# NikhilMukraj/spiking-neural-networks

Measured on AMD Instinct MI355X. Metric: neuron-steps/sec, higher is better.
Workload: dtype f32; 1 GPU; 256x256 Izhikevich lattice, dense gap-junction connectivity (all-to-all, x != y), dt=0.1, weights U[0.5,1.5]; neurons=65536, parallelism=single GPU

## Files before the change

### spiking-neural-networks_amd/csrc/snn_network_state.hpp

```cpp
#pragma once
#include <hip/hip_runtime.h>

#include <algorithm>
#include <atomic>
#include <cmath>
#include <cstdint>
#include <cstdio>
#include <cstdlib>
#include <cstring>
#include <map>
#include <memory>
#include <new>
#include <stdexcept>
#include <string>
#include <utility>
#include <vector>

#include "../../include/snn_amd.h"
#include "snn_kernels_connect.hpp"
#include "snn_kernels_connect_csr.hpp"
#include "snn_kernels_csr.hpp"
#include "snn_kernels_dense_step.hpp"
#include "snn_kernels_exchange.hpp"
#include "snn_kernels_graph_query.hpp"
// ... 128 lines not shown
    int plane;
    uint32_t pad;
    int dirties;
};

struct LatticeInfo {
    uint32_t id, rows, cols, first, count, slot;
    bool spike_train;
};

struct Cursors {
    long long clock = 0, run_step_offset = 0;
    uint64_t hist_steps = 0, hist_tick = 0;
};
struct CacheState {
    int shadow_cur = 0, cell_view_cur = 0;
    bool shadow_valid = false;
    bool view_dirty = true;
    bool counts_dirty = true, uni_dirty = true;
    uint32_t live_mask_applied = 0xFFFFFFFFu, n_live = K_TYPES, live_type[K_TYPES] = {0, 1, 2};
    uint32_t mirror_mask = 0xFFFFFFFFu;
};
struct Stats {
    struct Run { uint64_t launches = 0, steps = 0, stdp_steps = 0; } run;
    uint64_t run_fallbacks = 0, run_external_stream = 0;
    uint64_t direct_steps = 0, peer_steps = 0;
    uint64_t steps_dense_one_launch = 0, steps_dense_close = 0, steps_sparse_one_launch = 0, steps_sparse_image = 0;
    uint64_t steps_sparse_split = 0, steps_two_kernel = 0;
    uint64_t shadow_refreshes = 0, view_refreshes = 0, history_regrows = 0;
    uint64_t verify_runs = 0, verify_mismatches = 0, verify_skipped = 0;
};

}

struct snn_network {
    int device = 0;
    Options opt;
    Stats stat;
    Cursors cur;
    CacheState cache;
    hipStream_t stream = nullptr;
    hipStream_t own_stream = nullptr;
    bool external_stream = false;
    int model = 0, nt_kind = 0, rc_kind = 0, st_kind = 0;
    bool finalized = false;
    int electrical = 1, chemical = 0;

    hvec<LatticeInfo> lattices;
    hvec<LatticeInfo> st_lattices;
    hvec<long long> st_clock;
    hvec<float> stdp_host;
    hvec<uint32_t> plast_host;
    bool any_plasticity = false;
    std::map<uint32_t, bool> lattice_has_nt;
    bool any_nt_neurons = false, any_nt_cells = false;
    std::map<uint32_t, uint32_t> lattice_nt_mask;
    bool any_modulation = false;
    bool any_modulated = false;
    hvec<float> rm_host;
    hvec<uint32_t> rm_on_host;
    float *rm_dev = nullptr;
    uint32_t *rm_on_dev = nullptr;
    dev_ptr<float> trace;
    hvec<uint8_t> conn_kind_host;
    dev_ptr<uint8_t> conn_kind_dev;
    bool any_conn_kind = false;
    dev_ptr<float> pending;
    dev_ptr<float> edge_counter;
    dev_ptr<uint32_t> cross_bad;
    bool cross_checked = false;
    bool rstdp_pending = false;
    bool reward_since_defer = false;

    uint32_t nn = 0, nc = 0, n_tot = 0, n_pad = 0, c_pad = 0;
    uint32_t q0 = 0, q1 = 0, n_loc = 0, ld = 0, n_chunks = 0;
    XLayout xl{0};
    bool sharded = false;
    uint32_t n_shards = 1, shard_index = 0, shard_stride = 0;
    bool block_mode = false;
    hvec<uint32_t> lattice_slab;
    hvec<std::pair<uint32_t, uint32_t>> ranges;
    uint32_t n_owned = 0;
    hvec<uint32_t> owned_local_host;
    hvec<uint32_t> local_row_host;
    dev_ptr<uint32_t> own_block_dev, local_row_dev;
    dev_ptr<unsigned long long> own_mask_dev;
    RowMap rowmap{};
    bool x_dirty = true;
    bool x_agreed = false;
    bool refresh_agreed = false;
    int x_mode = SNN_EXCHANGE_ALLGATHER;
    uint32_t x_planes = 0, x_plane_id[WIRE_MAX_PLANES] = {0, 0, 0, 0};
    uint64_t x_block_words = 0;
    uint32_t *wire = nullptr;
    size_t wire_words = 0;
    hvec<hvec<uint32_t>> halo_need, halo_send;
    bool halo_committed = false;
    dev_ptr<uint32_t> halo_send_buf, halo_recv_buf, halo_send_idx, halo_recv_idx;
    hvec<uint64_t> x_send_off, x_send_words, x_recv_off, x_recv_words;
    dev_ptr<uint32_t> seg_count_dev[2], seg_first_dev[2];
    dev_ptr<uint64_t> seg_offset_dev[2], seg_loff_dev[2];
    uint32_t seg_n[2] = {0, 0}, seg_max[2] = {0, 0};
    dev_ptr<uint32_t> csr_border_dev, csr_interior_dev;
    uint32_t n_border = 0, n_interior = 0;
    dev_ptr<uint32_t> pack_ptr_dev, pack_segoff_dev, pack_count_dev, pack_index_dev;
    uint32_t recv_total = 0, send_bitmap_words = 0;
    bool send_bits_clean = true;
    bool update_packed = false;
    bool step_packed = false;
    bool interior_pending = false;
    dev_ptr<uint32_t> halo_send_buf2, halo_recv_buf2;
    dev_ptr<uint32_t> csr_plan_direct, halo_word_dev;
    bool direct_capable = false;
    bool peer_capable = false;
    bool direct_run = false;
    int hx_par = 0;
    bool stamp_pending = false;
    bool tail_done = false;
    dev_ptr<unsigned long long> p2p_recv[2];
    dev_ptr<uint32_t> p2p_flags;
    dev_ptr<uint32_t> p2p_done_blocks;
    pinned_ptr<uint32_t> p2p_failed;
    dev_ptr<uint32_t> agree_words_dev;
    uint32_t agree_words_cap = 0;
    uint64_t p2p_recv_words = 0;
    struct P2pPeer { uint64_t recv[2] = {0, 0}, flags = 0, recv_offset = 0; bool set = false; };
    hvec<P2pPeer> p2p_peers;
    dev_ptr<unsigned long long *> p2p_dst_dev[2];
    dev_ptr<uint32_t> p2p_peer_dev;
    dev_ptr<uint32_t *> p2p_signal_dev;
    uint32_t p2p_n_signal = 0;
    bool p2p_connected = false;
    hvec<dev_ptr<void>> p2p_retired;
    bool peer_run = false;
    uint32_t p2p_epoch = 0;
    hipStream_t comm_stream = nullptr;
    hipEvent_t ev_packed = nullptr, ev_exchanged = nullptr;

    struct Registered { dev_ptr<void> mem; size_t bytes; bool scratch; };
    hvec<Registered> registry;
    uint64_t registry_generation = 0;
    bool csr = false;
    uint64_t nnz = 0;
    dev_ptr<uint32_t> csr_ptr, csr_pre, csr_post, csr_t_ptr, csr_t_edge;
    dev_ptr<uint32_t> csr_row_len, csr_edge_slot;
    dev_ptr<float> csr_w;
    uint64_t sell_entries = 0;
    hvec<uint32_t> edge_slot_host;
    float *W = nullptr;
    dev_ptr<uint32_t> w24, w24_range;
    uint32_t w24_base = 0;
    bool w24_valid = false;
    bool w24_refused = false;
    bool w24_enabled = true;
    float *xbuf = nullptr;
    float *part_i = nullptr, *part_t = nullptr;
    uint32_t *n_in = nullptr, *tcount = nullptr;
    NeuronArrays na{};
    CellArrays ca{};
    uint32_t *lattice_slot = nullptr;
    float *stdp_dev = nullptr;
    uint32_t *plast_dev = nullptr;
    uint32_t *spike_list = nullptr, *spike_count = nullptr;
    hvec<uint32_t> cell_list_host;
    dev_ptr<uint32_t> cell_list_dev;
    uint32_t n_cells_listed = 0;
    dev_ptr<uint32_t> csr_plan;
    dev_ptr<uint32_t> csr_img_hdr, csr_plan_win;
    dev_ptr<uint4> csr_img_rec;
    uint64_t img_records = 0, img_staged_slices = 0;
    bool img_stale = true;
    dev_ptr<uint32_t> csr_img_hdr_direct, csr_plan_win_direct;
    dev_ptr<uint4> csr_img_rec_direct;
    uint64_t img_staged_slices_direct = 0;
    bool img_stale_direct = true;
    hvec<uint32_t> sell_pre_host, slice_ptr_host;
    uint2 *cell_view[2] = {nullptr, nullptr};
    bool cells_stepped = false;
    UniformTable *uni_neuron = nullptr, *uni_cell = nullptr;
    unsigned long long *run_granules = nullptr;
    unsigned long long *run_partials = nullptr;
    uint32_t run_tag = 1;
    float *run_w_out = nullptr;
    pinned_ptr<uint32_t> run_failed;
    uint32_t run_probed_grid = 0;
    CopyEntry *snap_table = nullptr;
    uint32_t *snap_buf = nullptr;
    uint32_t snap_entries = 0, snap_max_words = 0;
    uint64_t snap_registry_seen = 0;
    size_t snap_words = 0;
    hvec<CopyEntry> snap_table_host;
    size_t verify_words = 0;
    uint32_t *verify_buf = nullptr;
    dev_ptr<uint32_t> verify_report;
    pinned_ptr<char> copy_stage;
    dev_ptr<uint32_t> verify_third;
    size_t verify_third_words = 0;
    dev_ptr<char> verify_big;
    size_t verify_big_bytes = 0;
    uint64_t snap_generation = 0;
    std::string verify_text;
    struct Checkpoint {
        bool valid = false;
        hvec<std::pair<void *, hvec<uint8_t>>> arrays;
        hvec<long long> st_clock;
        Cursors cur;
        CacheState cache;
        uint32_t persistent_run = 1;
    } checkpoint;
    unsigned long long *run_timing = nullptr;
    unsigned long long run_timing_last[4] = {0, 0, 0, 0};
    uint32_t run_timing_steps = 0;
    bool stdp_pending = false;
    bool stdp_pending_rows_only = false;
    uint32_t *stdp_rowbits = nullptr;
    uint32_t *stdp_flag = nullptr;
    float *stdp_dcol = nullptr, *stdp_drow = nullptr;
    uint32_t dcol_stride = 0;
    long long *st_clock_dev = nullptr;
    pinned_ptr<long long> st_clock_pinned;
    bool run_active = false;
    float *shadow[2] = {nullptr, nullptr};
    uint32_t *tile_done = nullptr;
    uint32_t tile_done_len = 0;
    bool local_inputs_done = false;

    std::map<std::string, Attr> neuron_attrs, cell_attrs;

    int want_vhist = 0, want_raster = 0;
    int want_avg = 0, want_eeg = 0, want_counts = 0;
    hvec<int> want_whist;
    hvec<dev_ptr<float>> whist;
    bool any_whist = false;
    float eeg_ref = 0.007f, eeg_dist = 0.8f, eeg_cond = 251.0f;
    dev_ptr<float> summ_avg, summ_eeg;
    uint32_t *spike_counts = nullptr, *lat_first_dev = nullptr, *lat_count_dev = nullptr;
    uint64_t hist_cap = 0;
    hvec<hvec<float>> preset_host;
    dev_ptr<float> preset_times_dev;
    uint32_t hist_every = 1;
    dev_ptr<float> vhist, st_vhist;
    dev_ptr<unsigned long long> raster;

    uint64_t drive_seed = 0;
    uint32_t drive_threshold = 0;
    float drive_voltage = 0.0f;
    hvec<std::pair<hipEvent_t, hipEvent_t>> ev_pool_pl;
    size_t ev_used_pl = 0;
    uint64_t prof_launches_pl = 0;
    double prof_ms_pl = 0.0;
    int profile = 0;
    hvec<std::pair<hipEvent_t, hipEvent_t>> ev_pool;
    hvec<int> ev_counts;
    size_t ev_used = 0;
    uint64_t prof_launches = 0;
    double prof_ms = 0.0;
};

namespace {
static_assert(Options{}.run_resident_spin_limit == RUN_RESIDENT_SPIN_LIMIT, "snn_options.hpp restates the kernel header's default");

struct StatRow { const char *name; uint64_t (*read)(const snn_network &); };
#define STAT(field) [](const snn_network &n) -> uint64_t { return n.field; }
const StatRow STAT_TABLE[] = {
    {"persistent_run_launches", STAT(stat.run.launches)},
    {"persistent_run_steps", STAT(stat.run.steps)},
    {"persistent_run_stdp_steps", STAT(stat.run.stdp_steps)},
    {"persistent_run_fallbacks", STAT(stat.run_fallbacks)},
    {"persistent_run_external_stream", STAT(stat.run_external_stream)},
    {"halo_direct_steps", STAT(stat.direct_steps)},
    {"halo_peer_steps", STAT(stat.peer_steps)},
    {"steps_dense_one_launch", STAT(stat.steps_dense_one_launch)},
    {"steps_dense_close", STAT(stat.steps_dense_close)},
    {"steps_sparse_one_launch", STAT(stat.steps_sparse_one_launch)},
    {"steps_sparse_image", STAT(stat.steps_sparse_image)},
    {"steps_sparse_split", STAT(stat.steps_sparse_split)},
    {"steps_two_kernel", STAT(stat.steps_two_kernel)},
    {"shadow_refreshes", STAT(stat.shadow_refreshes)},
    {"view_refreshes", STAT(stat.view_refreshes)},
    {"history_regrows", STAT(stat.history_regrows)},
    {"verify_runs", STAT(stat.verify_runs)},
    {"verify_mismatches", STAT(stat.verify_mismatches)},
    {"verify_skipped", STAT(stat.verify_skipped)},
    {"image_staged_slices", STAT(img_staged_slices)},
    {"image_staged_slices_direct", STAT(img_staged_slices_direct)},
    {"run_timing_poll", STAT(run_timing_last[0])},
    {"run_timing_barrier", STAT(run_timing_last[1])},
    {"run_timing_turns", STAT(run_timing_last[2])},
    {"run_timing_update", STAT(run_timing_last[3])},
    {"run_timing_steps", STAT(run_timing_steps)},
};
#undef STAT

inline bool recording(const snn_network *net)
{
    return net->want_vhist || net->want_raster || net->want_avg || net->want_eeg || net->any_whist;
}
inline bool record_now(const snn_network *net)
{
    return recording(net) && net->cur.hist_tick % net->hist_every == 0;
}
}

namespace {

inline void w24_invalidate(snn_network *net) { net->w24_valid = false; net->w24_refused = false; }
// ... 783 lines not shown
```

### spiking-neural-networks_amd/csrc/snn_network_step.hpp

```cpp
#pragma once
#include "snn_dispatch.hpp"
#include "snn_network_state.hpp"

namespace {

enum ProfilePool { PROFILE_GRAPH_PASS, PROFILE_PLASTICITY };
int profile_open(snn_network *net, ProfilePool which, int passes, hipEvent_t *e1)
{
    *e1 = nullptr;
    if (!net->profile) return SNN_OK;
    auto &pool = which == PROFILE_PLASTICITY ? net->ev_pool_pl : net->ev_pool;
    size_t &used = which == PROFILE_PLASTICITY ? net->ev_used_pl : net->ev_used;
    if (used == pool.size()) {
        hipEvent_t x, y;
        HIP_TRY(hipEventCreate(&x), SNN_ERR_QUEUE);
        HIP_TRY(hipEventCreate(&y), SNN_ERR_QUEUE);
        pool.emplace_back(x, y);
    }
    if (which == PROFILE_GRAPH_PASS) {
        net->ev_counts.resize(pool.size(), 1);
        net->ev_counts[used] = passes;
    }
    const auto ev = pool[used++];
    *e1 = ev.second;
    HIP_TRY(hipEventRecord(ev.first, net->stream), SNN_ERR_QUEUE);
    return SNN_OK;
}
int profile_close(snn_network *net, hipEvent_t e1)
{
    if (e1) HIP_TRY(hipEventRecord(e1, net->stream), SNN_ERR_QUEUE);
    return SNN_OK;
}

uint32_t spike_train_args(snn_network *net, SpikeTrainArgs &a, int iterate, long long step_offset, long long view_clock)
{
    a = SpikeTrainArgs{};
    if (net->nc == 0) return 0;
    a.c = net->ca; a.n_cells = net->nc; a.st_kind = net->st_kind; a.nt_kind = net->nt_kind;
    a.iterate = iterate; a.lattice_clock = net->st_clock_dev; a.step_offset = step_offset;
    a.has_nt = net->any_nt_cells ? 1 : 0;
    a.view_clock = view_clock;
    a.vhist_row = (iterate && record_now(net) && net->want_vhist && net->st_vhist) ? net->st_vhist + (size_t)net->cur.hist_steps * net->c_pad : nullptr;
    a.cell_list = net->cell_list_dev; a.n_listed = net->n_cells_listed;
    const uint32_t work = net->cell_list_dev ? net->n_cells_listed : net->nc;
    if (work && net->cell_view[0]) {
        if (iterate) net->cache.cell_view_cur ^= 1;
        a.view_out = net->cell_view[net->cache.cell_view_cur];
    }
    return work;
}

int launch_spike_trains(snn_network *net, int iterate, long long step_offset, long long view_clock)
{
    SpikeTrainArgs a;
    const uint32_t work = spike_train_args(net, a, iterate, step_offset, view_clock);
    if (work == 0) return SNN_OK;
    hipLaunchKernelGGL(k_spike_trains, dim3((work + 255) / 256), dim3(256), 0, net->stream, a);
    HIP_TRY(hipGetLastError(), SNN_ERR_QUEUE);
    return SNN_OK;
}

enum InputsPart { INPUTS_ALL = 0, INPUTS_LOCAL = 1, INPUTS_REMOTE = 2 };
int flush_rstdp(snn_network *net);
int flush_stdp(snn_network *net);
bool fused_step_possible(const snn_network *net);

inline bool matrix_streamed(const snn_network *net)
{
    return !net->csr && (size_t)net->n_tot * net->ld * 4 > ((size_t)64 << 20);
}

bool stdp_deferral_applies(const snn_network *net)
{
    if (SNN_HAVE_CUSTOM_MODEL) return false;
    if (!net->opt.defer_stdp || !net->any_plasticity || net->any_modulation || net->any_whist || !matrix_streamed(net) || net->any_conn_kind ||
        net->lattices.size() > (size_t)STDP_MAX_LATTICES || net->n_loc == 0)
        return false;
    for (size_t l = 0; l < net->lattices.size(); ++l)
        if (net->stdp_host[l * PL_STRIDE + 5] != 0.0f) return false;
    return true;
}

StdpArgs stdp_args(snn_network *net)
{
    StdpArgs a{};
    a.W = net->W; a.ld = net->ld; a.n_loc = net->n_loc; a.q0 = net->q0; a.rows = net->rowmap; a.n_neurons = net->nn; a.n_tot = net->n_tot;
    a.xbuf = net->xbuf; a.xl = net->xl;
    a.last_firing_time = net->na.last_firing_time; a.st_last_firing_time = net->ca.last_firing_time;
    a.lattice_slot = net->lattice_slot; a.stdp = net->stdp_dev; a.do_plasticity = net->plast_dev;
    a.act = net->na.bcm_cur; a.avg = net->na.bcm_avg; a.st_act = net->ca.bcm_cur;
    a.spike_list = net->spike_list; a.spike_count = net->spike_count;
    a.flag = nullptr; a.dcol = net->stdp_dcol; a.drow = net->stdp_drow;
    a.dcol_stride = net->dcol_stride; a.n_lattices = (uint32_t)net->lattices.size();
    a.clock = net->cur.clock;
    a.conn_kind = net->any_conn_kind ? net->conn_kind_dev.get() : nullptr;
    a.st_lattice_slot = net->ca.lattice_slot;
    return a;
}
int ensure_exchange_plan(snn_network *net);
int launch_exchange_unpack(snn_network *net);

void local_chunks(const snn_network *net, uint32_t *begin, uint32_t *count)
{
    const uint32_t cb = (net->q0 + CHUNK - 1) / CHUNK, ce = net->q1 / CHUNK;
    *begin = cb;
    *count = ce > cb ? ce - cb : 0;
}

bool dense_close_applies(const snn_network *net);
bool w24_applies(const snn_network *net)
{
    return net->w24_enabled && !net->csr && !net->sharded && net->n_loc && net->n_tot && matrix_streamed(net) && net->electrical && !net->chemical &&
           !net->any_plasticity && !net->any_modulation && !net->any_conn_kind && !net->any_whist && !dense_close_applies(net);
}

int launch_inputs_dense(snn_network *net, InputsPart part, InputsArgs &a, uint32_t grid_chunks)
{
    const bool resident = (size_t)net->n_tot * net->ld * 4 <= ((size_t)64 << 20);
    const uint64_t waves4 = (uint64_t)((net->n_loc + 255) / 256) * grid_chunks;
    int shape = resident ? 0 : (waves4 < 57600 ? 2 : 1);
    if (net->opt.input_shape > 0 && !resident) shape = net->opt.input_shape;
    if (net->rstdp_pending && part != INPUTS_ALL) TRY(flush_rstdp(net));
    const bool stdp_fused = !LEAN_INPUT_PASS && net->stdp_pending && !net->rstdp_pending && part == INPUTS_ALL && shape != 0;
    if (net->stdp_pending && !stdp_fused) TRY(flush_stdp(net));
    auto in_shape = [&](auto SH, auto launch) {
        using S = InputsShape<decltype(SH)::value>;
        launch(dim3((net->n_loc + S::TILE - 1) / S::TILE, grid_chunks), dim3(S::THREADS));
    };
    if (stdp_fused) {
        net->stdp_pending = false;
        const bool rows_only = net->stdp_pending_rows_only;
        net->stdp_pending_rows_only = false;
        a.W_rw = net->W; a.stdp_count = net->spike_count; a.stdp_flag = net->stdp_flag;
        a.stdp_dcol = net->stdp_dcol; a.stdp_drow = net->stdp_drow; a.lattice_slot = net->lattice_slot;
        a.dcol_stride = net->dcol_stride; a.n_lattices = (uint32_t)net->lattices.size();
        a.stdp_rowbits = net->stdp_rowbits;
        for (int k = 0; k < K_TYPES; ++k) a.live_type[k] = (uint32_t)k;
        for_synapses(net->electrical, net->chemical, [&](auto E, auto C) {
            if constexpr (!LEAN_INPUT_PASS)
                for_value<1, 2>(shape, [&](auto SH) {
                    in_shape(SH, [&](dim3 grid, dim3 block) {
                        if (rows_only) hipLaunchKernelGGL((k_inputs_dense<E(), C(), SH(), K_TYPES, 2>), grid, block, 0, net->stream, a);
                        else hipLaunchKernelGGL((k_inputs_dense<E(), C(), SH(), K_TYPES, 1>), grid, block, 0, net->stream, a);
                    });
                });
        });
    } else if (net->rstdp_pending) {
        net->rstdp_pending = false;
        RstdpInputsArgs ra{};
        ra.in = a; ra.W = net->W; ra.C = net->trace;
        ra.last_firing_time = net->na.last_firing_time; ra.lattice_slot = net->lattice_slot;
        ra.rm = net->rm_dev; ra.rm_on = net->rm_on_dev;
        ra.dop = net->reward_since_defer ? RM_DOPAMINE_BEFORE : RM_DOPAMINE;
        for_synapses(net->electrical, net->chemical, [&](auto E, auto C) {
            for_value<1, 2, 0>(shape, [&](auto SH) {
                in_shape(SH, [&](dim3 grid, dim3 block) {
                    hipLaunchKernelGGL((k_inputs_rstdp<E(), C(), SH()>), grid, block, 0, net->stream, ra);
                });
            });
        });
    } else if (net->w24_valid && net->w24 && part == INPUTS_ALL && shape != 0 && net->electrical && !net->chemical) {
        const v4u *image = reinterpret_cast<const v4u *>(net->w24.get());
        const uint32_t base = net->w24_base;
        for_value<1, 2>(shape, [&](auto SH) {
            in_shape(SH, [&](dim3 grid, dim3 block) {
                hipLaunchKernelGGL((k_inputs_dense_w24<true, SH()>), grid, block, 0, net->stream, a, image, base);
            });
        });
    } else {
        if (LEAN_INPUT_PASS && net->chemical)
            for (int k = 0; k < K_TYPES; ++k) a.live_type[k] = (uint32_t)k;
        for_synapses(net->electrical, net->chemical, [&](auto E, auto C) {
            for_value<1, 2, 0>(shape, [&](auto SH) {
                in_shape(SH, [&](dim3 grid, dim3 block) {
                    auto pass = [&](auto NT) { hipLaunchKernelGGL((k_inputs_dense<E(), C(), SH(), NT()>), grid, block, 0, net->stream, a); };
                    if constexpr (!C() || LEAN_INPUT_PASS) pass(int_c<3>{});
                    else for_value<1, 2, 3>((int)net->cache.n_live, pass);
                });
            });
        });
    }
    return SNN_OK;
}

int launch_inputs(snn_network *net, InputsPart part = INPUTS_ALL)
{
    if (net->n_loc == 0 || net->n_tot == 0) return SNN_OK;
    uint32_t lc_begin = 0, lc_count = 0;
    local_chunks(net, &lc_begin, &lc_count);
    uint32_t grid_chunks = net->n_chunks;
    InputsArgs a{};
    a.chunk_first = 0; a.hole_begin = net->n_chunks; a.hole_count = 0;
    if (part == INPUTS_LOCAL) { a.chunk_first = lc_begin; grid_chunks = lc_count; }
    if (part == INPUTS_REMOTE) { a.hole_begin = lc_begin; a.hole_count = lc_count; grid_chunks = net->n_chunks - lc_count; }
    if (grid_chunks == 0) return SNN_OK;
    a.W = net->W; a.ld = net->ld; a.n_loc = net->n_loc; a.q0 = net->q0; a.rows = net->rowmap; a.n_neurons = net->nn; a.n_tot = net->n_tot;
    a.xbuf = net->xbuf; a.xl = net->xl; a.gap_conductance = net->na.gap_conductance; a.uni = net->uni_neuron;
    a.st_value = net->ca.presyn_value; a.st_last_firing_time = net->ca.last_firing_time;
    a.st_view = net->cell_view[net->cache.cell_view_cur];
    a.st_nt_t = net->ca.nt_t; a.st_nt_flags = net->ca.nt_flags; a.c_pad = net->c_pad;
    a.nt_flags = net->na.nt_flags; a.n_pad = net->n_pad;
    a.part_i = net->part_i; a.part_t = net->part_t; a.n_chunks = net->n_chunks;
    for (int k = 0; k < K_TYPES; ++k) a.live_type[k] = net->cache.live_type[k];
    hipEvent_t e1 = nullptr;
    TRY(profile_open(net, PROFILE_GRAPH_PASS, (part == INPUTS_LOCAL && lc_count < net->n_chunks) ? 0 : 1, &e1));
    if (net->csr && net->csr_ptr) {
        CsrInputsArgs ca{};
        ca.g = csr_graph(net);
        ca.in = a;
        const dim3 g((((net->n_loc + 63) / 64) * 64 + 255) / 256);
        for_synapses(net->electrical, net->chemical, [&](auto E, auto C) {
            hipLaunchKernelGGL((k_inputs_csr<E(), C()>), g, dim3(256), 0, net->stream, ca);
        });
    } else if (net->csr) {
        HIP_TRY(hipMemsetAsync(net->part_i, 0, (size_t)net->ld * 4, net->stream), SNN_ERR_BUFFER_WRITE);
        HIP_TRY(hipMemsetAsync(net->part_t, 0, (size_t)K_TYPES * net->ld * 4, net->stream), SNN_ERR_BUFFER_WRITE);
    } else {
        TRY(launch_inputs_dense(net, part, a, grid_chunks));
    }
    HIP_TRY(hipGetLastError(), SNN_ERR_QUEUE);
    return profile_close(net, e1);
}

int launch_update(snn_network *net)
{
    if (net->n_loc == 0) return SNN_OK;
    UpdateArgs a{};
    a.n = net->na;
    a.part_i = net->part_i; a.part_t = net->part_t; a.n_in = net->n_in; a.tcount = net->tcount;
    a.ld = net->ld; a.n_chunks = net->n_tot ? net->n_chunks : 0; a.q0 = net->q0; a.n_loc = net->n_loc; a.rows = net->rowmap;
    a.clock = net->cur.clock;
    a.electrical = net->electrical; a.chemical = net->chemical; a.nt_kind = net->nt_kind; a.rc_kind = net->rc_kind;
    a.vhist_row = (record_now(net) && net->want_vhist && net->vhist) ? net->vhist + (size_t)net->cur.hist_steps * net->n_pad : nullptr;
    a.spike_row = (record_now(net) && net->want_raster && net->raster) ? net->raster + (size_t)net->cur.hist_steps * (net->n_pad / 64) : nullptr;
    a.spike_counts = net->want_counts ? net->spike_counts : nullptr;
    a.xout = net->xbuf; a.xout2 = nullptr;
    a.has_nt = net->any_nt_neurons ? 1 : 0;
    a.live_mask = net->cache.live_mask_applied;
    a.bcm = net->model == SNN_MODEL_BCM_IZHIKEVICH;
    a.model_is_custom = net->model == SNN_MODEL_CUSTOM;
    net->update_packed = false;
    if (net->sharded && !net->csr && net->opt.update_packs && !net->x_dirty && net->x_mode == SNN_EXCHANGE_ALLGATHER &&
        net->wire && net->x_block_words && net->n_loc <= net->shard_stride) {
        a.wire_out = net->wire + (size_t)net->shard_index * net->x_block_words;
        a.wire_count = net->shard_stride; a.wire_planes = net->x_planes;
        for (uint32_t s = 0; s < net->x_planes; ++s) a.wire_plane_id[s] = net->x_plane_id[s];
        net->update_packed = true;
    }
    net->cache.shadow_valid = false;
    const uint32_t ub = 256u;
    dim3 grid((net->ld + ub - 1) / ub);
    const bool all_planes = net->opt.update_all_planes && net->chemical && !net->csr && net->model != SNN_MODEL_CUSTOM;
    const bool wide = all_planes && net->opt.update_all_planes >= 2 && a.n_chunks >= 4 && (a.n_chunks + 3) / 4 <= 32;
    TouchList touch{};
    if (wide) {
        grid = dim3(net->ld / 64);
        auto add = [&](const void *p) {
            if (!p || touch.n_neuron >= 56) return;
            for (uint32_t i = 0; i < touch.n_neuron; ++i) if (touch.by_neuron[i] == p) return;
            touch.by_neuron[touch.n_neuron++] = static_cast<const uint32_t *>(p);
        };
        for (const auto &kv : net->neuron_attrs) {
            const Attr &at = kv.second;
            if (at.store == S_PLAIN) add(at.base);
            else if (at.store == S_PLAIN_K)
                for (int k = 0; k < K_TYPES; ++k) if (a.live_mask >> k & 1u) add(static_cast<const uint32_t *>(at.base) + (size_t)k * at.pad);
        }
        for (int pl : {PLANE_V, PLANE_SPIKE}) add(net->xbuf + net->xl.at(0, pl));
        for (int k = 0; k < K_TYPES; ++k) if (a.live_mask >> k & 1u) add(net->xbuf + net->xl.at(0, PLANE_T0 + k));
        touch.by_column[touch.n_column++] = net->n_in;
        for (int k = 0; k < K_TYPES; ++k) if (a.live_mask >> k & 1u) touch.by_column[touch.n_column++] = net->tcount + (size_t)k * net->ld;
        if (net->opt.update_all_planes == 3) touch.n_neuron = touch.n_column = 0;
    }
    for_model(UpdateModels{}, net->model, [&](auto M) {
        if constexpr (M() == CUSTOM_MODEL) hipLaunchKernelGGL((k_update<M(), false>), grid, dim3(ub), 0, net->stream, a);
        else if (wide) hipLaunchKernelGGL((k_update_wide<M()>), grid, dim3(256), 0, net->stream, a, touch);
        else if (all_planes) hipLaunchKernelGGL((k_update<M(), true>), grid, dim3(ub), 0, net->stream, a);
        else hipLaunchKernelGGL((k_update<M(), false>), grid, dim3(ub), 0, net->stream, a);
    });
    HIP_TRY(hipGetLastError(), SNN_ERR_QUEUE);
    return SNN_OK;
}

int launch_plasticity_kernels(snn_network *net);

int launch_plasticity(snn_network *net)
{
    if (!net->any_plasticity || net->nn == 0) return SNN_OK;
    hipEvent_t e1 = nullptr;
    TRY(profile_open(net, PROFILE_PLASTICITY, 1, &e1));
    TRY(launch_plasticity_kernels(net));
    return profile_close(net, e1);
}

bool stdp_small_applies(const snn_network *net)
{
    if (!net->opt.stdp_small || net->csr || net->sharded || net->n_tot > 1024u || net->n_loc != net->nn || net->nn == 0) return false;
    for (size_t l = 0; l < net->lattices.size(); ++l)
        if (net->stdp_host[l * PL_STRIDE + 5] != 0.0f) return false;
    return true;
}

int launch_plasticity_kernels(snn_network *net)
{
    StdpArgs a = stdp_args(net);
    if (stdp_small_applies(net)) {
        hipLaunchKernelGGL(k_stdp_small, dim3(16), dim3(1024), 0, net->stream, a);
        HIP_TRY(hipGetLastError(), SNN_ERR_QUEUE);
        return SNN_OK;
    }
    const bool defer = stdp_deferral_applies(net);
    if (defer) a.flag = net->stdp_flag;
    HIP_TRY(hipMemsetAsync(net->spike_count, 0, 4, net->stream), SNN_ERR_BUFFER_WRITE);
    hipLaunchKernelGGL(k_spike_compact, dim3((net->nn + 255) / 256), dim3(256), 0, net->stream, a);
// ... 22 lines not shown
        ca.g = csr_graph(net);
        ca.s = a;
        net->img_stale = net->img_stale_direct = true;
        hipLaunchKernelGGL(k_stdp_csr_in, dim3(1024), dim3(64), 0, net->stream, ca);
        HIP_TRY(hipGetLastError(), SNN_ERR_QUEUE);
        hipLaunchKernelGGL(k_stdp_csr_out, dim3(1024), dim3(64), 0, net->stream, ca);
        HIP_TRY(hipGetLastError(), SNN_ERR_QUEUE);
        return SNN_OK;
    }
    const unsigned sy = 64;
    if (net->opt.stdp_columns_form == 1) {
        const uint32_t groups = (net->n_tot + 3u) / 4u;
        const unsigned slabs = std::max(1u, std::min(1024u, groups / 16u));
        hipLaunchKernelGGL(k_stdp_columns_quads, dim3(4, slabs), dim3(256), 0, net->stream, a);
    } else {
        hipLaunchKernelGGL(k_stdp_columns, dim3((net->n_tot + 255) / 256, sy), dim3(256), 0, net->stream, a);
    }
    HIP_TRY(hipGetLastError(), SNN_ERR_QUEUE);
    hipLaunchKernelGGL(k_stdp_rows, dim3((net->n_loc + 255) / 256, sy), dim3(256), 0, net->stream, a);
    HIP_TRY(hipGetLastError(), SNN_ERR_QUEUE);
    return SNN_OK;
}

bool fused_step_possible(const snn_network *net)
{
    const bool compiled = !SNN_HAVE_CUSTOM_MODEL || (SNN_HAVE_CUSTOM_NEURON && net->model == SNN_MODEL_CUSTOM);
    return compiled && net->opt.fused_step && !net->csr && !net->sharded && !net->drive_threshold && net->n_loc && net->n_tot &&
           net->n_chunks <= RESIDENT_MAX_CHUNKS && (size_t)net->n_tot * net->ld * 4 <= ((size_t)64 << 20);
}

int launch_rstdp_pass(snn_network *net, int dop)
{
    if (net->csr) {
        if (!net->csr_ptr) return SNN_OK;
        CsrRewardArgs a{};
        a.g = csr_graph(net); a.c = net->trace; a.q0 = net->q0; a.rows = net->rowmap; a.n_neurons = net->nn;
        a.last_firing_time = net->na.last_firing_time; a.lattice_slot = net->lattice_slot;
        a.rm = net->rm_dev; a.rm_on = net->rm_on_dev; a.dop = dop;
        net->img_stale = net->img_stale_direct = true;
        hipLaunchKernelGGL(k_rstdp_csr, dim3((net->n_loc + 255) / 256), dim3(256), 0, net->stream, a);
        HIP_TRY(hipGetLastError(), SNN_ERR_QUEUE);
        return SNN_OK;
    }
    RewardArgs a{};
    a.W = net->W; a.C = net->trace; a.ld = net->ld; a.n_loc = net->n_loc; a.q0 = net->q0; a.n_neurons = net->nn;
    a.last_firing_time = net->na.last_firing_time; a.lattice_slot = net->lattice_slot;
    a.rm = net->rm_dev; a.rm_on = net->rm_on_dev; a.dop = dop;
    const unsigned gx = (net->n_loc + 255) / 256;
    const unsigned gy = std::max(1u, std::min<unsigned>((net->nn + 3) / 4, std::max(1u, 8192u / gx)));
    hipLaunchKernelGGL(k_rstdp_dense, dim3(gx, gy), dim3(256), 0, net->stream, a);
    HIP_TRY(hipGetLastError(), SNN_ERR_QUEUE);
    return SNN_OK;
}

static RewardCrossArgs reward_cross_args(snn_network *net)
{
    RewardCrossArgs a{};
    a.s = stdp_args(net);
    a.s.conn_kind = net->conn_kind_dev;
    a.C = net->trace; a.P = net->pending; a.K = net->edge_counter;
    a.rm = net->rm_dev; a.rm_on = net->rm_on_dev; a.bad = net->cross_bad;
    return a;
}

int launch_reward_cross(snn_network *net)
{
    if (!net->any_conn_kind || net->nn == 0 || !net->trace || !net->pending) return SNN_OK;
    if (net->csr) {
        if (!net->csr_ptr || net->n_loc == 0) return SNN_OK;
        CsrRewardCrossArgs c{};
        c.g = csr_graph(net);
        c.r = reward_cross_args(net);
        net->img_stale = net->img_stale_direct = true;
        hipLaunchKernelGGL(k_reward_cross_csr, dim3((net->n_loc + 255) / 256), dim3(256), 0, net->stream, c);
        HIP_TRY(hipGetLastError(), SNN_ERR_QUEUE);
        return SNN_OK;
    }
    const unsigned gx = (net->nn + 255) / 256;
    const unsigned gy = std::max(1u, std::min<unsigned>(net->n_tot, std::max(1u, 16384u / gx)));
    hipLaunchKernelGGL(k_reward_cross, dim3(gx, gy), dim3(256), 0, net->stream, reward_cross_args(net));
    HIP_TRY(hipGetLastError(), SNN_ERR_QUEUE);
    return SNN_OK;
}

int check_reward_cross(snn_network *net)
{
    if (!net->any_conn_kind || net->cross_checked || net->nn == 0 || !net->pending) return SNN_OK;
    HIP_TRY(hipMemsetAsync(net->cross_bad, 0, 4, net->stream), SNN_ERR_BUFFER_WRITE);
    const unsigned gx = (net->nn + 255) / 256;
    const unsigned gy = std::max(1u, std::min<unsigned>(net->n_tot, std::max(1u, 16384u / gx)));
    if (net->csr) {
        if (net->csr_ptr && net->n_loc) {
            CsrRewardCrossArgs c{};
            c.g = csr_graph(net);
            c.r = reward_cross_args(net);
            hipLaunchKernelGGL(k_reward_cross_check_csr, dim3((net->n_loc + 255) / 256), dim3(256), 0, net->stream, c);
        }
    } else {
        hipLaunchKernelGGL(k_reward_cross_check, dim3(gx, gy), dim3(256), 0, net->stream, reward_cross_args(net));
    }
    HIP_TRY(hipGetLastError(), SNN_ERR_QUEUE);
    uint32_t bad = 0;
    HIP_TRY(hipMemcpyAsync(&bad, net->cross_bad, 4, hipMemcpyDeviceToHost, net->stream), SNN_ERR_BUFFER_READ);
    HIP_TRY(hipStreamSynchronize(net->stream), SNN_ERR_WAIT);
    static const char *why[] = {"", "a connection of a visited lattice has no reverse connection of the same kind: the reference's outgoing half "
        "looks the reverse connection up and unwraps it (neuron/mod.rs:4768-4771, 4929-4932)",
        "reward-modulated weights where no side has a modulator, or from a spike train into a plastic plain lattice (neuron/mod.rs:4743, 4789)",
        "plain weights between a plastic plain lattice and a reward-modulated one (neuron/mod.rs:4729-4733, 4778)",
        "a BCM lattice on a connection of a reward-modulated network (the reference's network has one plasticity rule)"};
    if (bad) return fail(SNN_ERR_BAD_STATE, why[bad < 5 ? bad : 1]);
    net->cross_checked = true;
    return SNN_OK;
}

int launch_reward_modulation(snn_network *net)
{
    if (!net->any_modulation || net->nn == 0 || net->n_loc == 0 || !net->trace) return SNN_OK;
    if (!net->csr && net->opt.defer_rstdp && !net->any_whist && !fused_step_possible(net)) {
        net->rstdp_pending = true;
        net->reward_since_defer = false;
        return SNN_OK;
    }
    return launch_rstdp_pass(net, RM_DOPAMINE);
}

int flush_stdp(snn_network *net)
{
    if (!net->stdp_pending) return SNN_OK;
    net->stdp_pending = false;
    if (net->n_loc == 0 || net->nn == 0) { net->stdp_pending_rows_only = false; return SNN_OK; }
    StdpArgs a = stdp_args(net);
    const unsigned sy = 64;
    if (net->stdp_pending_rows_only) {
        net->stdp_pending_rows_only = false;
    } else {
        hipLaunchKernelGGL(k_stdp_apply_columns, dim3((net->n_tot + 255) / 256, sy), dim3(256), 0, net->stream, a);
        HIP_TRY(hipGetLastError(), SNN_ERR_QUEUE);
    }
    hipLaunchKernelGGL(k_stdp_apply_rows, dim3((net->n_loc + 255) / 256, sy), dim3(256), 0, net->stream, a);
    HIP_TRY(hipGetLastError(), SNN_ERR_QUEUE);
    return SNN_OK;
}

int flush_rstdp(snn_network *net)
{
    if (!net->rstdp_pending) return SNN_OK;
    net->rstdp_pending = false;
    return launch_rstdp_pass(net, net->reward_since_defer ? RM_DOPAMINE_BEFORE : RM_DOPAMINE);
}

int time_input_pass(snn_network *net, float *ms)
{
    *ms = 0.0f;
    hipEvent_t e0 = nullptr, e1 = nullptr;
    if (hipEventCreate(&e0) != hipSuccess || hipEventCreate(&e1) != hipSuccess) return fail(SNN_ERR_QUEUE, "hipEventCreate failed");
    const size_t bytes = (size_t)net->n_tot * net->ld * 4;
    const int passes = bytes < ((size_t)4 << 30) ? 8 : 1;
    int rc = launch_inputs(net);
    if (rc == SNN_OK && hipEventRecord(e0, net->stream) != hipSuccess) rc = fail(SNN_ERR_QUEUE, "hipEventRecord failed");
    for (int i = 0; i < passes && rc == SNN_OK; ++i) rc = launch_inputs(net);
    if (rc == SNN_OK && (hipEventRecord(e1, net->stream) != hipSuccess || hipEventSynchronize(e1) != hipSuccess ||
                         hipEventElapsedTime(ms, e0, e1) != hipSuccess))
        rc = fail(SNN_ERR_WAIT, "placement timing failed");
    *ms /= (float)passes;
    (void)hipEventDestroy(e0);
    (void)hipEventDestroy(e1);
    return rc;
}

int choose_matrix_placement(snn_network *net)
{
    const size_t count = net->csr ? 0 : wcount(net->n_tot, net->ld);
    const size_t bytes = count * sizeof(float);
    if (bytes >= ((size_t)1 << 30) && net->n_loc) {
        const int prof = net->profile;
        net->profile = 0;
        float best_ms = 0.0f;
        int rc = time_input_pass(net, &best_ms);
        hvec<dev_ptr<void>> losers;
        for (int cand = 0; cand < 4 && rc == SNN_OK; ++cand) {
            size_t free_b = 0, total_b = 0;
            dev_ptr<void> b;
            if (hipMemGetInfo(&free_b, &total_b) != hipSuccess || free_b < bytes + (bytes >> 2) ||
                alloc_streamed(&b, bytes) != hipSuccess)
                break;
            float *a = net->W;
            float ms_b = 0.0f;
            net->W = static_cast<float *>(b.get());
            rc = time_input_pass(net, &ms_b);
            if (getenv("SNN_DEBUG_PLACEMENT"))
                fprintf(stderr, "[snn] matrix placement: held %p %.3f ms, candidate %p %.3f ms\n", (void *)a, best_ms, b.get(), ms_b);
            if (rc == SNN_OK && ms_b < best_ms * 0.99f) {
                losers.push_back(dev_replace(net, a, std::move(b)));
                w24_invalidate(net);
                best_ms = ms_b;
            } else {
                net->W = a;
                losers.push_back(std::move(b));
            }
        }
        net->profile = prof;
        if (rc != SNN_OK) return rc;
    }
    if (count) {
        hipLaunchKernelGGL(k_fill_u32, dim3(4096), dim3(256), 0, net->stream,
                           reinterpret_cast<uint32_t *>(net->W), count, 0x7FC00000u);
        HIP_TRY(hipGetLastError(), SNN_ERR_QUEUE);
        HIP_TRY(hipStreamSynchronize(net->stream), SNN_ERR_WAIT);
    }
    return SNN_OK;
}

int ensure_w24(snn_network *net)
{
    if (!w24_applies(net)) {
        net->w24 = nullptr;
        w24_invalidate(net);
        return SNN_OK;
    }
    if (net->w24_valid || net->w24_refused) return SNN_OK;
    auto refuse = [&]() { (void)hipGetLastError(); net->w24 = nullptr; net->w24_refused = true; return SNN_OK; };
    if (!net->w24_range && snn_malloc(&net->w24_range, 256) != hipSuccess) return refuse();
    uint32_t range[2] = {0xFFFFFFFFu, 0u};
    HIP_TRY(copy_sync(net, net->w24_range, range, 8, hipMemcpyHostToDevice), SNN_ERR_BUFFER_WRITE);
    hipLaunchKernelGGL(k_w24_range, dim3(4096), dim3(256), 0, net->stream, net->W, net->ld, net->n_loc, net->n_tot, net->w24_range.get());
    HIP_TRY(hipGetLastError(), SNN_ERR_QUEUE);
    HIP_TRY(copy_sync(net, range, net->w24_range, 8, hipMemcpyDeviceToHost), SNN_ERR_BUFFER_READ);
    if (!w24_encodable(range[0], range[1])) return refuse();
    const size_t bytes = w24_image_bytes(net->n_tot, net->ld);
    if (!net->w24 && alloc_streamed(&net->w24, bytes) != hipSuccess) return refuse();
    net->w24_base = w24_base(range[0], range[1]);
    hipLaunchKernelGGL(k_w24_pack, dim3((net->ld + 255) / 256, (unsigned)w24_row_units(net->n_tot)), dim3(256), 0, net->stream,
                       net->W, net->ld, net->n_loc, net->n_tot, net->w24_base, reinterpret_cast<w24_v4u *>(net->w24.get()));
    HIP_TRY(hipGetLastError(), SNN_ERR_QUEUE);
    net->w24_valid = true;
    if (bytes >= ((size_t)1 << 30)) {
        const int prof = net->profile;
        net->profile = 0;
        float best_ms = 0.0f;
        int rc = time_input_pass(net, &best_ms);
        hvec<dev_ptr<uint32_t>> losers;
        for (int cand = 0; cand < 2 && rc == SNN_OK; ++cand) {
            size_t free_b = 0, total_b = 0;
            dev_ptr<uint32_t> b;
            if (hipMemGetInfo(&free_b, &total_b) != hipSuccess || free_b < bytes + (bytes >> 2) || alloc_streamed(&b, bytes) != hipSuccess) {
                (void)hipGetLastError();
                break;
            }
            if (hipMemcpyAsync(b, net->w24, bytes, hipMemcpyDeviceToDevice, net->stream) != hipSuccess) { losers.push_back(std::move(b)); break; }
            std::swap(net->w24, b);
            float ms_b = 0.0f;
            rc = time_input_pass(net, &ms_b);
            if (getenv("SNN_DEBUG_PLACEMENT"))
                fprintf(stderr, "[snn] image placement: held %p %.3f ms, candidate %p %.3f ms\n", (void *)b.get(), best_ms, (void *)net->w24.get(), ms_b);
            if (rc == SNN_OK && ms_b < best_ms * 0.99f) best_ms = ms_b;
            else std::swap(net->w24, b);
            losers.push_back(std::move(b));
        }
        net->profile = prof;
        if (rc != SNN_OK) return rc;
    }
    return SNN_OK;
}

bool fused_step_applies(const snn_network *net)
{
    return fused_step_possible(net) && !net->local_inputs_done;
}

int fused_step_args(snn_network *net, InputsArgs &a, UpdateArgs &u, bool in_place = false)
{
    const size_t xelems = (size_t)NUM_PLANES * net->xl.stride;
    if (in_place) {
        net->cache.shadow_valid = false;
    } else if (!net->shadow[0]) {
        TRY(dev_alloc_t(net, &net->shadow[0], xelems));
        TRY(dev_alloc_t(net, &net->shadow[1], xelems));
        net->cache.shadow_valid = false;
    }
    if (!in_place && !net->cache.shadow_valid) {
        for (int i = 0; i < 2; ++i)
            HIP_TRY(hipMemcpyAsync(net->shadow[i], net->xbuf, xelems * 4, hipMemcpyDeviceToDevice, net->stream),
                    SNN_ERR_BUFFER_WRITE);
        net->cache.shadow_valid = true;
        net->stat.shadow_refreshes += 1;
    }
    float *cur = in_place ? net->xbuf : net->shadow[net->cache.shadow_cur];
    float *next = in_place ? nullptr : net->shadow[net->cache.shadow_cur ^ 1];
    a = InputsArgs{};
    a.chunk_first = 0; a.hole_begin = net->n_chunks; a.hole_count = 0;
    a.W = net->W; a.ld = net->ld; a.n_loc = net->n_loc; a.q0 = net->q0; a.rows = net->rowmap; a.n_neurons = net->nn; a.n_tot = net->n_tot;
    a.xbuf = cur; a.xl = net->xl; a.gap_conductance = net->na.gap_conductance; a.uni = net->uni_neuron;
    a.st_value = net->ca.presyn_value; a.st_last_firing_time = net->ca.last_firing_time;
    a.st_view = net->cell_view[net->cache.cell_view_cur];
    a.st_nt_t = net->ca.nt_t; a.st_nt_flags = net->ca.nt_flags; a.c_pad = net->c_pad;
    a.nt_flags = net->na.nt_flags; a.n_pad = net->n_pad;
    a.part_i = net->part_i; a.part_t = net->part_t; a.n_chunks = net->n_chunks;
    for (int k = 0; k < K_TYPES; ++k) a.live_type[k] = (uint32_t)k;
    u = UpdateArgs{};
    u.n = net->na;
    u.n.xbuf = cur;
    u.part_i = net->part_i; u.part_t = net->part_t; u.n_in = net->n_in; u.tcount = net->tcount;
    u.ld = net->ld; u.n_chunks = net->n_chunks; u.q0 = net->q0; u.n_loc = net->n_loc; u.rows = net->rowmap;
    u.clock = net->cur.clock;
    u.electrical = net->electrical; u.chemical = net->chemical; u.nt_kind = net->nt_kind; u.rc_kind = net->rc_kind;
    u.vhist_row = (record_now(net) && net->want_vhist && net->vhist) ? net->vhist + (size_t)net->cur.hist_steps * net->n_pad : nullptr;
    u.spike_row = (record_now(net) && net->want_raster && net->raster) ? net->raster + (size_t)net->cur.hist_steps * (net->n_pad / 64) : nullptr;
    u.spike_counts = net->want_counts ? net->spike_counts : nullptr;
    u.xout = net->xbuf; u.xout2 = next;
    u.has_nt = net->any_nt_neurons ? 1 : 0;
    u.live_mask = net->cache.live_mask_applied;
    u.bcm = net->model == SNN_MODEL_BCM_IZHIKEVICH;
    u.model_is_custom = net->model == SNN_MODEL_CUSTOM;
    return SNN_OK;
}

int launch_step_resident(snn_network *net)
{
    ResidentArgs r{};
    TRY(fused_step_args(net, r.in, r.up));
    hipEvent_t e1 = nullptr;
    TRY(profile_open(net, PROFILE_GRAPH_PASS, 1, &e1));
    const bool quarters = net->opt.resident_quarters && net->n_chunks <= 2 && net->n_tot > 64;
    const dim3 grid((net->n_loc + 63) / 64), block(64 * net->n_chunks * (quarters ? 4 : 1));
    for_model(ResidentStepModels{}, net->model, [&](auto M) {
        for_synapses(net->electrical, net->chemical, [&](auto E, auto C) {
            if (quarters) hipLaunchKernelGGL((k_step_resident_q<M(), E(), C()>), grid, block, 0, net->stream, r);
            else hipLaunchKernelGGL((k_step_resident<M(), E(), C()>), grid, block, 0, net->stream, r);
        });
    });
    HIP_TRY(hipGetLastError(), SNN_ERR_QUEUE);
    TRY(profile_close(net, e1));
    net->cache.shadow_cur ^= 1;
    return SNN_OK;
}

bool dense_close_applies(const snn_network *net)
{
    return !SNN_HAVE_CUSTOM_MODEL && net->opt.dense_close && !net->csr && !net->sharded && !net->drive_threshold && net->n_loc && net->n_tot &&
           net->n_loc == net->nn && net->electrical && matrix_streamed(net) && !net->local_inputs_done && !net->stdp_pending &&
           !net->rstdp_pending && net->opt.input_shape == 0 && net->n_chunks <= net->opt.dense_close_max_chunks;
}

int launch_dense_close(snn_network *net)
{
    DenseStepArgs r{};
    TRY(fused_step_args(net, r.in, r.up));
    const uint64_t waves4 = (uint64_t)((net->n_loc + 255) / 256) * net->n_chunks;
    const int shape = waves4 < 57600 ? 2 : 1;
    const uint32_t tiles = shape == 1 ? (net->n_loc + InputsShape<1>::TILE - 1) / InputsShape<1>::TILE
                                      : (net->n_loc + InputsShape<2>::TILE - 1) / InputsShape<2>::TILE;
    if (net->tile_done_len < tiles) {
        net->tile_done = nullptr;
        TRY(dev_alloc_t(net, &net->tile_done, (size_t)tiles));
        HIP_TRY(memset_sync(net, net->tile_done, 0, (size_t)tiles * 4), SNN_ERR_BUFFER_WRITE);
        net->tile_done_len = tiles;
        TRY(fused_step_args(net, r.in, r.up));
    }
    r.tile_done = net->tile_done;
    const bool one_type = net->chemical && net->cache.n_live == 1;
    if (one_type) for (int k = 0; k < K_TYPES; ++k) r.in.live_type[k] = net->cache.live_type[k];
    hipEvent_t e1 = nullptr;
    TRY(profile_open(net, PROFILE_GRAPH_PASS, 1, &e1));
    const dim3 grid(tiles, net->n_chunks), block(256);
    for_model(FusedModels{}, net->model, [&](auto M) {
        for_value<1, 2>(shape, [&](auto SH) {
            if (!net->chemical) hipLaunchKernelGGL((k_inputs_dense_close<M(), true, false, SH(), 3>), grid, block, 0, net->stream, r);
            else if (one_type) hipLaunchKernelGGL((k_inputs_dense_close<M(), true, true, SH(), 1>), grid, block, 0, net->stream, r);
            else hipLaunchKernelGGL((k_inputs_dense_close<M(), true, true, SH(), 3>), grid, block, 0, net->stream, r);
        });
    });
    HIP_TRY(hipGetLastError(), SNN_ERR_QUEUE);
    TRY(profile_close(net, e1));
    net->cache.shadow_cur ^= 1;
    return SNN_OK;
}

bool run_resident_shape(const snn_network *net);
bool run_resident_stdp_ok(const snn_network *net);
int launch_plasticity(snn_network *net);
bool run_resident_applies(const snn_network *net)
{
    return run_resident_shape(net) && !net->external_stream;
}
bool run_resident_stdp_ok(const snn_network *net)
{
    if (!net->opt.persistent_stdp || net->chemical || net->nc || net->n_tot > RUN_RESIDENT_GROUP_ROWS || net->any_conn_kind || net->opt.defer_stdp ||
        net->lattices.size() > RUN_STDP_MAX_LATTICES)
        return false;
    for (size_t l = 0; l < net->lattices.size(); ++l)
        if (net->plast_host[l] && net->stdp_host[l * PL_STRIDE + 5] != 0.0f) return false;
    return true;
}
bool run_resident_shape(const snn_network *net)
{
    const bool chem_ok = !net->chemical || (net->n_tot <= RUN_RESIDENT_GROUP_ROWS && net->opt.persistent_chem &&
                                            net->nt_kind != SNN_NT_CUSTOM && net->rc_kind != SNN_RC_CUSTOM);
    return !SNN_HAVE_CUSTOM_MODEL && net->opt.fused_step && !net->csr && !net->sharded && !net->drive_threshold && net->n_loc &&
           net->opt.persistent_run && net->n_loc == net->nn && net->nn + net->nc == net->n_tot &&
           (net->nc == 0 || ((net->st_kind == SNN_ST_POISSON || net->st_kind == SNN_ST_RATE) && !net->any_nt_cells &&
                             !net->cell_list_dev && !SNN_HAVE_CUSTOM_REFRACTORINESS)) &&
           net->n_tot <= RUN_RESIDENT_MAX_NEURONS && (net->electrical || net->chemical) && chem_ok &&
           (!net->any_plasticity || run_resident_stdp_ok(net)) &&
           !net->any_modulation && !net->any_whist && !net->want_avg && !net->want_eeg && net->hist_every == 1 &&
           net->model != SNN_MODEL_BCM_IZHIKEVICH && !net->local_inputs_done;
}

constexpr size_t RUN_GRANULE_WORDS = (size_t)2 * RUN_GRANULE_PLANES * RUN_RESIDENT_MAX_NEURONS;
constexpr size_t RUN_PARTIAL_WORDS = (size_t)2 * RUN_RESIDENT_MAX_TILES * (RUN_RESIDENT_MAX_GROUPS - 1) * 256;

int run_snapshot(snn_network *net, bool restore)
{
    if (!restore && (!net->snap_table || net->snap_registry_seen != net->registry_generation)) {
// ... 568 lines not shown
```

Before: 33.13 million neuron-steps/s.

## Widen packed-weight image placement search and allow image in sharded and partial passes

Enables the packed 24-bit weight image for sharded networks and for partial input passes, not only full passes. The placement search now tries up to five candidate allocations instead of two. Each candidate is timed as the minimum over several individually recorded passes rather than an average, and the search runs only once per allocation. The aim is to stream a smaller weight image more often and to land it at a faster physical placement, at the cost of longer setup and more transient memory use.

```diff
diff --git a/profiles/measure_first_run.py b/profiles/measure_first_run.py
--- /dev/null
+++ b/profiles/measure_first_run.py
@@ -0,0 +1,21 @@
+import json, os, sys, time
+ROOT = os.path.dirname(os.path.dirname(os.path.abspath(__file__)))
+sys.path.insert(0, ROOT)
+import numpy as np
+import snn_amd
+from snn_amd import synthetic
+n = 256 * 256
+t0 = time.perf_counter()
+dn = snn_amd.DeviceNetwork(model=snn_amd.IZHIKEVICH, device=0)
+dn.add_lattice(0, 256, 256)
+dn.finalize()
+t_fin = time.perf_counter() - t0
+dn.set_attr(0, "gap_conductance", np.full(n, 10.0, np.float32))
+dn.set_attr(0, "current_voltage", synthetic.uniform(1, n, -65.0, 30.0))
+dn.fill_graph_synthetic(2, 0.5, 1.5, with_diagonal=False)
+dn.synchronize()
+t0 = time.perf_counter(); dn.run(5); dn.synchronize(); first = time.perf_counter() - t0
+t0 = time.perf_counter(); dn.run(5); dn.synchronize(); second = time.perf_counter() - t0
+print(json.dumps({"lib": "SNN_AMD_LIB" if "SNN_AMD_LIB" in os.environ else "in-tree", "finalize_s": round(t_fin, 4), "first_run_5_steps_s": round(first, 4),
+                  "second_run_5_steps_s": round(second, 4), "bytes_per_synapse": dn.input_kernel_bytes() / (n * (n))}))
+dn.close()
diff --git a/spiking-neural-networks_amd/csrc/snn_network_state.hpp b/spiking-neural-networks_amd/csrc/snn_network_state.hpp
--- a/spiking-neural-networks_amd/csrc/snn_network_state.hpp
+++ b/spiking-neural-networks_amd/csrc/snn_network_state.hpp
@@ -304,6 +304,7 @@
     uint32_t w24_base = 0;
     bool w24_valid = false;
     bool w24_refused = false;
+    bool w24_placed = false;
     bool w24_enabled = true;
     float *xbuf = nullptr;
     float *part_i = nullptr, *part_t = nullptr;
diff --git a/spiking-neural-networks_amd/csrc/snn_network_step.hpp b/spiking-neural-networks_amd/csrc/snn_network_step.hpp
--- a/spiking-neural-networks_amd/csrc/snn_network_step.hpp
+++ b/spiking-neural-networks_amd/csrc/snn_network_step.hpp
@@ -1,4 +1,5 @@
 #pragma once
+#include <chrono>
 #include "snn_dispatch.hpp"
 #include "snn_network_state.hpp"
 
@@ -110,7 +111,7 @@
 bool dense_close_applies(const snn_network *net);
 bool w24_applies(const snn_network *net)
 {
-    return net->w24_enabled && !net->csr && !net->sharded && net->n_loc && net->n_tot && matrix_streamed(net) && net->electrical && !net->chemical &&
+    return net->w24_enabled && !net->csr && net->n_loc && net->n_tot && matrix_streamed(net) && net->electrical && !net->chemical &&
            !net->any_plasticity && !net->any_modulation && !net->any_conn_kind && !net->any_whist && !dense_close_applies(net);
 }
 
@@ -159,7 +160,7 @@
                 });
             });
         });
-    } else if (net->w24_valid && net->w24 && part == INPUTS_ALL && shape != 0 && net->electrical && !net->chemical) {
+    } else if (net->w24_valid && net->w24 && shape != 0 && net->electrical && !net->chemical) {
         const v4u *image = reinterpret_cast<const v4u *>(net->w24.get());
         const uint32_t base = net->w24_base;
         for_value<1, 2>(shape, [&](auto SH) {
@@ -488,19 +489,36 @@
 int time_input_pass(snn_network *net, float *ms)
 {
     *ms = 0.0f;
-    hipEvent_t e0 = nullptr, e1 = nullptr;
-    if (hipEventCreate(&e0) != hipSuccess || hipEventCreate(&e1) != hipSuccess) return fail(SNN_ERR_QUEUE, "hipEventCreate failed");
-    const size_t bytes = (size_t)net->n_tot * net->ld * 4;
-    const int passes = bytes < ((size_t)4 << 30) ? 8 : 1;
-    int rc = launch_inputs(net);
-    if (rc == SNN_OK && hipEventRecord(e0, net->stream) != hipSuccess) rc = fail(SNN_ERR_QUEUE, "hipEventRecord failed");
-    for (int i = 0; i < passes && rc == SNN_OK; ++i) rc = launch_inputs(net);
-    if (rc == SNN_OK && (hipEventRecord(e1, net->stream) != hipSuccess || hipEventSynchronize(e1) != hipSuccess ||
-                         hipEventElapsedTime(ms, e0, e1) != hipSuccess))
-        rc = fail(SNN_ERR_WAIT, "placement timing failed");
-    *ms /= (float)passes;
-    (void)hipEventDestroy(e0);
-    (void)hipEventDestroy(e1);
+    const bool image = net->w24_valid && net->w24;
+    const size_t bytes = image ? w24_image_bytes(net->n_tot, net->ld) : (size_t)net->n_tot * net->ld * 4;
+    const int passes = bytes < ((size_t)4 << 30) ? 8 : 5;
+    const bool debug = getenv("SNN_DEBUG_PLACEMENT") != nullptr;
+    hvec<std::pair<hipEvent_t, hipEvent_t>> ev;
+    int rc = SNN_OK;
+    for (int i = 0; i < passes && rc == SNN_OK; ++i) {
+        hipEvent_t e0 = nullptr, e1 = nullptr;
+        if (hipEventCreate(&e0) != hipSuccess || hipEventCreate(&e1) != hipSuccess) rc = fail(SNN_ERR_QUEUE, "hipEventCreate failed");
+        if (e0 || e1) ev.emplace_back(e0, e1);
+    }
+    if (rc == SNN_OK) rc = launch_inputs(net);
+    for (int i = 0; i < passes && rc == SNN_OK; ++i) {
+        if (hipEventRecord(ev[i].first, net->stream) != hipSuccess) rc = fail(SNN_ERR_QUEUE, "hipEventRecord failed");
+        if (rc == SNN_OK) rc = launch_inputs(net);
+        if (rc == SNN_OK && hipEventRecord(ev[i].second, net->stream) != hipSuccess) rc = fail(SNN_ERR_QUEUE, "hipEventRecord failed");
+    }
+    if (rc == SNN_OK && hipEventSynchronize(ev[passes - 1].second) != hipSuccess) rc = fail(SNN_ERR_WAIT, "placement timing failed");
+    for (int i = 0; i < passes && rc == SNN_OK; ++i) {
+        float t = 0.0f;
+        if (hipEventElapsedTime(&t, ev[i].first, ev[i].second) != hipSuccess) { rc = fail(SNN_ERR_WAIT, "placement timing failed"); break; }
+        if (debug) fprintf(stderr, "[snn] placement pass %d over %s %p: %.3f ms\n", i, image ? "the image" : "W",
+                           image ? (void *)net->w24.get() : (void *)net->W, t);
+        if (i == 0 || t < *ms) *ms = t;
+    }
+    if (rc != SNN_OK) (void)hipStreamSynchronize(net->stream);
+    for (const auto &e : ev) {
+        if (e.first) (void)hipEventDestroy(e.first);
+        if (e.second) (void)hipEventDestroy(e.second);
+    }
     return rc;
 }
 
@@ -564,22 +582,32 @@
     HIP_TRY(copy_sync(net, range, net->w24_range, 8, hipMemcpyDeviceToHost), SNN_ERR_BUFFER_READ);
     if (!w24_encodable(range[0], range[1])) return refuse();
     const size_t bytes = w24_image_bytes(net->n_tot, net->ld);
-    if (!net->w24 && alloc_streamed(&net->w24, bytes) != hipSuccess) return refuse();
+    if (!net->w24) {
+        if (alloc_streamed(&net->w24, bytes) != hipSuccess) return refuse();
+        net->w24_placed = false;
+    }
     net->w24_base = w24_base(range[0], range[1]);
     hipLaunchKernelGGL(k_w24_pack, dim3((net->ld + 255) / 256, (unsigned)w24_row_units(net->n_tot)), dim3(256), 0, net->stream,
                        net->W, net->ld, net->n_loc, net->n_tot, net->w24_base, reinterpret_cast<w24_v4u *>(net->w24.get()));
     HIP_TRY(hipGetLastError(), SNN_ERR_QUEUE);
     net->w24_valid = true;
-    if (bytes >= ((size_t)1 << 30)) {
+    if (bytes >= ((size_t)1 << 30) && !net->local_inputs_done && !net->w24_placed) {
         const int prof = net->profile;
         net->profile = 0;
         float best_ms = 0.0f;
         int rc = time_input_pass(net, &best_ms);
         hvec<dev_ptr<uint32_t>> losers;
-        for (int cand = 0; cand < 2 && rc == SNN_OK; ++cand) {
+        using clk = std::chrono::steady_clock;
+        const bool debug = getenv("SNN_DEBUG_PLACEMENT") != nullptr;
+        const clk::time_point t_search = clk::now();
+        double alloc_s = 0.0;
+        for (int cand = 0; cand < 5 && rc == SNN_OK; ++cand) {
             size_t free_b = 0, total_b = 0;
             dev_ptr<uint32_t> b;
-            if (hipMemGetInfo(&free_b, &total_b) != hipSuccess || free_b < bytes + (bytes >> 2) || alloc_streamed(&b, bytes) != hipSuccess) {
+            const clk::time_point t_alloc = clk::now();
+            const bool got = hipMemGetInfo(&free_b, &total_b) == hipSuccess && free_b >= bytes + (bytes >> 2) && alloc_streamed(&b, bytes) == hipSuccess;
+            alloc_s += std::chrono::duration<double>(clk::now() - t_alloc).count();
+            if (!got) {
                 (void)hipGetLastError();
                 break;
             }
@@ -587,14 +615,22 @@
             std::swap(net->w24, b);
             float ms_b = 0.0f;
             rc = time_input_pass(net, &ms_b);
-            if (getenv("SNN_DEBUG_PLACEMENT"))
+            if (debug)
                 fprintf(stderr, "[snn] image placement: held %p %.3f ms, candidate %p %.3f ms\n", (void *)b.get(), best_ms, (void *)net->w24.get(), ms_b);
             if (rc == SNN_OK && ms_b < best_ms * 0.99f) best_ms = ms_b;
             else std::swap(net->w24, b);
             losers.push_back(std::move(b));
         }
+        const clk::time_point t_free = clk::now();
+        const size_t n_losers = losers.size();
+        losers.clear();
+        if (debug)
+            fprintf(stderr, "[snn] image placement: %zu further allocations of %.2f GB, search %.3f s of which allocating %.3f s, freeing %.3f s\n",
+                    n_losers, (double)bytes * 1e-9, std::chrono::duration<double>(clk::now() - t_search).count(), alloc_s,
+                    std::chrono::duration<double>(clk::now() - t_free).count());
         net->profile = prof;
         if (rc != SNN_OK) return rc;
+        net->w24_placed = true;
     }
     return SNN_OK;
 }
```

Result: no change. 33.06 million neuron-steps/s (-0.2%).
